# RoozbehSanaei/Structure-from-Motion-3D-Reconstruction

Hardware: NVIDIA B200
Metric: KLT feature-tracks/sec (+ RANSAC hyp*pts/sec under 'ransac') (higher is better)
Workload: dtype f64

## Files before the change

structure-from-motion-3d-reconstruction_b200/csrc/klt_lane.cu:

```cuda
#include "common.cuh"

namespace {

constexpr int LR = 5;
constexpr int LN = 2 * LR + 4;
constexpr int LNC = 2 * LR + 3;
constexpr int LIMG = LN * 16;
constexpr int LSTRIDE = 2 * LIMG + 16;
constexpr int LWARPS = 1;

__device__ __forceinline__ double byte_f64(uint32_t w, int k) {
  const uint32_t b = __byte_perm(w, 0, 0x4440 | k);
  double d;
  asm("cvt.rn.f64.u32 %0, %1;" : "=d"(d) : "r"(b));
  return d;
}

__device__ __forceinline__ void row_bytes(const uint4 q, double (&v)[LN]) {
  const uint32_t w[4] = {q.x, q.y, q.z, q.w};
#pragma unroll
  for (int i = 0; i < LN; i++) v[i] = byte_f64(w[i >> 2], i & 3);
}

template <int I0, int I1>
__device__ __forceinline__ void hlerp_row(const unsigned char* rowp, double fx, double (&h)[LNC]) {
  double px[LN];
  row_bytes(*reinterpret_cast<const uint4*>(rowp), px);
#pragma unroll
  for (int i = I0; i < I1; i++) h[i] = __fma_rn(fx, px[i + 1] - px[i], px[i]);
}

template <int ACC, bool MASKED>
__device__ __forceinline__ void walk_row(const unsigned char* tile, int v, double fx, double fy, unsigned cm, unsigned rm,
                                         double (&h1p)[LNC], double (&h0p)[LNC], const double (&sold)[LNC], const double (&smid)[LNC],
                                         double (&snew)[LNC], double (&acc)[ACC][5]) {
  double px[LN];
  row_bytes(*reinterpret_cast<const uint4*>(tile + v * 16), px);
  const unsigned cnew = MASKED ? (((rm >> (v - 1)) & 1u) ? cm : 0u) : 0u;
  const unsigned cpix = MASKED ? (((rm >> (v - 2)) & 1u) ? cm : 0u) : 0u;
#pragma unroll
  for (int i = 0; i < LNC; i++) {
    const double h = __fma_rn(fx, px[i + 1] - px[i], px[i]);
    double sn = __fma_rn(fy, h - h1p[i], h1p[i]);
    if (MASKED) sn = ((cnew >> i) & 1u) ? sn : 0.0;
    snew[i] = sn;
    h1p[i] = h;
  }
  row_bytes(*reinterpret_cast<const uint4*>(tile + LIMG + (v - 1) * 16), px);
#pragma unroll
  for (int i = 1; i <= LNC - 2; i++) {
    const double h = __fma_rn(fx, px[i + 1] - px[i], px[i]);
    double s0 = __fma_rn(fy, h - h0p[i], h0p[i]);
    if (MASKED) s0 = ((cpix >> i) & 1u) ? s0 : 0.0;
    h0p[i] = h;
    const double gx2 = smid[i + 1] - smid[i - 1];
    const double gy2 = snew[i] - sold[i];
    const double e = s0 - smid[i];
    double(&a)[5] = acc[i % ACC];
    a[0] = __fma_rn(gx2, gx2, a[0]);
    a[1] = __fma_rn(gx2, gy2, a[1]);
    a[2] = __fma_rn(gy2, gy2, a[2]);
    a[3] = __fma_rn(gx2, e, a[3]);
    a[4] = __fma_rn(gy2, e, a[4]);
  }
}

template <int ACC, bool MASKED>
__device__ __forceinline__ void window_sums(const unsigned char* tile, double fx, double fy, unsigned cm, unsigned rm, double& a00,
                                            double& a01, double& a11, double& b0, double& b1) {
  double h1p[LNC], h0p[LNC], s0[LNC], s1[LNC], s2[LNC], t[LNC];
  double acc[ACC][5];
#pragma unroll
  for (int j = 0; j < ACC; j++)
#pragma unroll
    for (int q = 0; q < 5; q++) acc[j][q] = 0.0;
  hlerp_row<0, LNC>(tile, fx, h1p);
  hlerp_row<0, LNC>(tile + 16, fx, t);
  const unsigned c0 = MASKED ? ((rm & 1u) ? cm : 0u) : 0u, c1 = MASKED ? ((rm & 2u) ? cm : 0u) : 0u;
#pragma unroll
  for (int i = 0; i < LNC; i++) {
    s0[i] = __fma_rn(fy, t[i] - h1p[i], h1p[i]);
    if (MASKED) s0[i] = ((c0 >> i) & 1u) ? s0[i] : 0.0;
    h1p[i] = t[i];
  }
  hlerp_row<0, LNC>(tile + 32, fx, t);
#pragma unroll
  for (int i = 0; i < LNC; i++) {
    s1[i] = __fma_rn(fy, t[i] - h1p[i], h1p[i]);
    if (MASKED) s1[i] = ((c1 >> i) & 1u) ? s1[i] : 0.0;
    h1p[i] = t[i];
  }
  hlerp_row<1, LNC - 1>(tile + LIMG + 16, fx, h0p);
#pragma unroll 1
  for (int v = 3; v < LN; v += 3) {
    walk_row<ACC, MASKED>(tile, v, fx, fy, cm, rm, h1p, h0p, s0, s1, s2, acc);
    walk_row<ACC, MASKED>(tile, v + 1, fx, fy, cm, rm, h1p, h0p, s1, s2, s0, acc);
    if (v + 2 < LN) walk_row<ACC, MASKED>(tile, v + 2, fx, fy, cm, rm, h1p, h0p, s2, s0, s1, acc);
  }
  a00 = acc[0][0]; a01 = acc[0][1]; a11 = acc[0][2]; b0 = acc[0][3]; b1 = acc[0][4];
#pragma unroll
  for (int j = 1; j < ACC; j++) {
    a00 += acc[j][0]; a01 += acc[j][1]; a11 += acc[j][2]; b0 += acc[j][3]; b1 += acc[j][4];
  }
}

struct StageRegs {
  uint4 lo, hi;
};

template <bool CLAMP>
__device__ __forceinline__ void stage_load(StageRegs& r, const uint8_t* __restrict__ imgA, const uint8_t* __restrict__ imgB, int pitch,
                                           int h, int x0, int y0, int lane) {
  const int img = lane >= LN ? 1 : 0, row = lane - img * LN;
  int y = y0 + row;
  if (CLAMP) y = y < 0 ? 0 : (y > h - 1 ? h - 1 : y);
  const uint8_t* rowp = (img ? imgA : imgB) + (size_t)y * pitch;
  const int xa = x0 & ~15, o = x0 & 15;
  int c0 = xa, c1 = xa + 16;
  if (CLAMP) {
    c0 = c0 < 0 ? 0 : (c0 > pitch - 16 ? pitch - 16 : c0);
    c1 = c1 < 0 ? 0 : (c1 > pitch - 16 ? pitch - 16 : c1);
  }
  r.lo = __ldg(reinterpret_cast<const uint4*>(rowp + c0));
  r.hi = make_uint4(0, 0, 0, 0);
  if (o > 2) r.hi = __ldg(reinterpret_cast<const uint4*>(rowp + c1));
}

__device__ __forceinline__ void stage_store(const StageRegs& r, unsigned char* tile_s, int x0, int lane) {
  const int img = lane >= LN ? 1 : 0, row = lane - img * LN;
  const int o = x0 & 15, q = o >> 2, sh = (o & 3) * 8;
  uint32_t W[8] = {r.lo.x, r.lo.y, r.lo.z, r.lo.w, r.hi.x, r.hi.y, r.hi.z, r.hi.w};
  if (q & 2) { W[0] = W[2]; W[1] = W[3]; W[2] = W[4]; W[3] = W[5]; W[4] = W[6]; W[5] = W[7]; }
  if (q & 1) { W[0] = W[1]; W[1] = W[2]; W[2] = W[3]; W[3] = W[4]; W[4] = W[5]; }
  uint4 out;
  out.x = __funnelshift_r(W[0], W[1], sh);
  out.y = __funnelshift_r(W[1], W[2], sh);
  out.z = __funnelshift_r(W[2], W[3], sh);
  out.w = __funnelshift_r(W[3], W[4], sh);
  *reinterpret_cast<uint4*>(tile_s + img * LIMG + row * 16) = out;
}

template <int ACC, int MINB, int LSTAGE, bool MASKED>
__global__ void __launch_bounds__(32 * LWARPS, MINB) klt_lane_kernel(KltLaunch k, const int* __restrict__ in_list,
                                                                     const int* __restrict__ in_count, int* __restrict__ defer_count,
                                                                     int* __restrict__ defer_list) {
  extern __shared__ __align__(16) unsigned char smem_raw[];
  const unsigned FULL = 0xffffffffu;
  const int warp = threadIdx.x >> 5, lane = threadIdx.x & 31;
  unsigned char* wtile = smem_raw + (size_t)warp * 32 * LSTRIDE;
  unsigned char* tile = wtile + lane * LSTRIDE;
  const long long total = (long long)k.npairs * k.cap;
  const long long nwork = MASKED ? (long long)*in_count : total;
  for (long long wbase = ((long long)blockIdx.x * LWARPS + warp) * 32; wbase < nwork; wbase += (long long)gridDim.x * LWARPS * 32) {
  const long long widx = wbase + lane;
  long long g = widx;
  if (MASKED) g = widx < nwork ? (long long)in_list[widx] : total;
  const int pair = g < total ? (int)(g / k.cap) : 0;
  const int slot = (int)(g - (long long)pair * k.cap);
  const bool valid = g < total && (!k.counts || slot < k.counts[pair]);

  double2 p0 = make_double2(0.0, 0.0);
  if (valid) p0 = k.p0[g];
  double px = p0.x, py = p0.y, x1 = 0.0, y1 = 0.0;
  int n_it = 0;
  bool alive = valid;
  const int ndir = k.pb ? 2 : 1;

  for (int dir = 0; dir < ndir; dir++) {
    for (int l = k.pv.levels - 1; l >= 0; --l) {
      const int w = k.pv.w[l], h = k.pv.h[l], pitch = k.pv.pitch[l];
      const uint8_t* lbase = k.pv.base[l];
      const size_t fstride = k.pv.fstride[l];
      const double scale = 1.0 / (double)(1 << l);
      const double plx = px * scale, ply = py * scale;
      double dlx = 0.0, dly = 0.0;
      bool done = !alive;
      int tFX = INT_MIN, tFY = INT_MIN;
      for (int it = 0; it < k.iters; ++it) {
        if (!__any_sync(FULL, !done)) break;
        const double x = plx + dlx, y = ply + dly;
        const double fxx = floor(x), fyy = floor(y);
        int FX = 0, FY = 0;
        unsigned cm = 0, rm = 0;
        bool act = !done;
        if (act) {
          const bool finite_ok = (fabs(fxx) < 1.0e9) && (fabs(fyy) < 1.0e9);
          FX = finite_ok ? (int)fxx : 0;
          FY = finite_ok ? (int)fyy : 0;
          bool ok;
          if (!MASKED) {
            ok = finite_ok && FX - LR - 1 >= 0 && FX + LR + 3 <= w - 1 && FY - LR - 1 >= 0 && FY + LR + 3 <= h - 1;
          } else {
            const double lim = 1.0 - 5.9604644775390625e-8;
            ok = finite_ok && w >= 16 && h >= 16 && (x - fxx) <= lim && (y - fyy) <= lim;
            if (ok) {
#pragma unroll
              for (int i = 0; i < LNC; i++) {
                const int cx = FX + i - LR - 1, cy = FY + i - LR - 1;
                cm |= (cx >= 0 && cx <= w - 2) ? (1u << i) : 0u;
                rm |= (cy >= 0 && cy <= h - 2) ? (1u << i) : 0u;
              }
            }
          }
          if (!ok) {
            alive = false;
            done = true;
            act = false;
          }
        }
        unsigned need = __ballot_sync(FULL, act && (FX != tFX || FY != tFY));
        if (need) {
          __syncwarp();
          while (need) {
            int ss[LSTAGE], sx0[LSTAGE];
            StageRegs sr[LSTAGE];
#pragma unroll
            for (int j = 0; j < LSTAGE; j++) {
              ss[j] = need ? __ffs(need) - 1 : -1;
              need &= need - 1;
              const int src = ss[j] < 0 ? 0 : ss[j];
              const int sFX = __shfl_sync(FULL, FX, src), sFY = __shfl_sync(FULL, FY, src), spair = __shfl_sync(FULL, pair, src);
              const int sA = k.fa0 + spair * k.fa_step, sB = k.fb0 + spair * k.fb_step;
              sx0[j] = sFX - LR - 1;
              if (ss[j] >= 0 && lane < 2 * LN)
                stage_load<MASKED>(sr[j], lbase + (size_t)(dir ? sB : sA) * fstride, lbase + (size_t)(dir ? sA : sB) * fstride, pitch, h,
                                   sx0[j], sFY - LR - 1, lane);
            }
#pragma unroll
            for (int j = 0; j < LSTAGE; j++)
              if (ss[j] >= 0 && lane < 2 * LN) stage_store(sr[j], wtile + ss[j] * LSTRIDE, sx0[j], lane);
          }
          __syncwarp();
        }
        if (act) {
          tFX = FX;
          tFY = FY;
          double a00, a01, a11, b0, b1;
          window_sums<ACC, MASKED>(tile, x - fxx, y - fyy, cm, rm, a00, a01, a11, b0, b1);
          double sx = 0.0, sy = 0.0;
          const double det = a00 * a11 - a01 * a01;
          if (!(fabs(det) < 16.0 * 1e-9)) {
            const double rd = 2.0 / det;
            sx = (a11 * b0 - a01 * b1) * rd;
            sy = (a00 * b1 - a01 * b0) * rd;
          }
          n_it++;
          dlx += sx;
          dly += sy;
          if (sfm_lk_step_small(sx, sy)) done = true;
        }
      }
      const double up = (double)(1 << l);
      px = (plx + dlx) * up;
      py = (ply + dly) * up;
    }
    if (dir == 0) {
      x1 = px;
      y1 = py;
    }
  }
  if (alive) {
    k.p1[g] = make_double2(x1, y1);
    if (k.pb) k.pb[g] = make_double2(px, py);
    if (k.nit) k.nit[g] = n_it;
    if (k.keep) {
      const double fbd = hypot(px - p0.x, py - p0.y);
      k.keep[g] = (fbd >= k.fb_thresh) ? 0 : 1;
    }
  }
  const unsigned dm = __ballot_sync(FULL, valid && !alive);
  if (dm) {
    int base = 0;
    if (lane == 0) base = atomicAdd(defer_count, __popc(dm));
    base = __shfl_sync(FULL, base, 0);
    if (valid && !alive) defer_list[base + __popc(dm & ((1u << lane) - 1u))] = (int)g;
  }
  __syncwarp();
  }
}


constexpr int QM = 50;
static_assert(QM * 8 <= 2 * LIMG, "the matrices alias the lane's tile");

template <typename T>
struct QuadFam {
  T m[10];
};

__device__ __forceinline__ int qmad(int a, int b, int c) { return a * b + c; }
__device__ __forceinline__ float qmad(float a, float b, float c) { return __fmaf_rn(a, b, c); }

template <bool SYM, typename T>
__device__ __forceinline__ void quad_same_row(QuadFam<T>& f, const T (&a)[12], const T (&b)[12], bool first, bool last) {
  const T p1 = a[0] * b[0], p12 = a[11] * b[11];
  T mid = a[1] * b[1];
#pragma unroll
  for (int c = 2; c < 11; c++) mid = qmad(a[c], b[c], mid);
  const T left = mid + p1, right = mid + p12;
  T rs01 = a[0] * b[1];
  if (!SYM) rs01 = qmad(b[0], a[1], rs01);
#pragma unroll
  for (int c = 1; c < 11; c++) {
    rs01 = qmad(a[c], b[c + 1], rs01);
    if (!SYM) rs01 = qmad(b[c], a[c + 1], rs01);
  }
  const T zero = (T)0;
  f.m[0] += last ? zero : left;
  f.m[4] += last ? zero : right;
  f.m[1] += last ? zero : rs01;
  f.m[7] += first ? zero : left;
  f.m[9] += first ? zero : right;
  f.m[8] += first ? zero : rs01;
}

template <bool SYM, typename T>
__device__ __forceinline__ void quad_cross_row(QuadFam<T>& f, const T (&ap)[12], const T (&bp)[12], const T (&ac)[12],
                                               const T (&bc)[12]) {
  T q1 = ap[0] * bc[0], q12 = ap[11] * bc[11], mid = ap[1] * bc[1];
  if (!SYM) {
    q1 = qmad(bp[0], ac[0], q1);
    q12 = qmad(bp[11], ac[11], q12);
    mid = qmad(bp[1], ac[1], mid);
  }
#pragma unroll
  for (int c = 2; c < 11; c++) {
    mid = qmad(ap[c], bc[c], mid);
    if (!SYM) mid = qmad(bp[c], ac[c], mid);
  }
  f.m[2] += mid + q1;
  f.m[6] += mid + q12;
  T m03 = f.m[3], m12 = f.m[5];
#pragma unroll
  for (int c = 0; c < 11; c++) {
    m03 = qmad(ap[c], bc[c + 1], m03);
    m12 = qmad(ap[c + 1], bc[c], m12);
    if (!SYM) {
      m03 = qmad(bp[c], ac[c + 1], m03);
      m12 = qmad(bp[c + 1], ac[c], m12);
    }
  }
  f.m[3] = m03;
  f.m[5] = m12;
}

template <bool SYM, typename T>
__device__ __forceinline__ void quad_store(const QuadFam<T>& f, double* m) {
#pragma unroll
  for (int e = 0; e < 10; e++) {
    const bool diag = e == 0 || e == 4 || e == 7 || e == 9;
    const double v = (double)f.m[e];
    m[e] = (SYM && !diag) ? v + v : v;
  }
}

__device__ __forceinline__ void row_vals(const uint4 q, int (&v)[LN]) {
  const uint32_t w[4] = {q.x, q.y, q.z, q.w};
#pragma unroll
  for (int i = 0; i < LN; i++) v[i] = (int)__byte_perm(w[i >> 2], 0, 0x4440 | (i & 3));
}
__device__ __forceinline__ void row_vals(const uint4 q, float (&v)[LN]) {
  const uint32_t w[4] = {q.x, q.y, q.z, q.w};
#pragma unroll
  for (int i = 0; i < LN; i++) v[i] = __uint_as_float(__byte_perm(w[i >> 2], 0x4B000000u, 0x7650 | (i & 3)));
}

template <typename T, int PASS>
__device__ __forceinline__ void quad_sweep(const unsigned char* tile, QuadFam<T>& f0, QuadFam<T>& f1, QuadFam<T>& f2) {
  constexpr bool NX = PASS != 2, NY = PASS != 1, NE = PASS != 0;
  T dxp[12], dyp[12], dep[12];
#pragma unroll
  for (int c = 0; c < 12; c++) dxp[c] = dyp[c] = dep[c] = (T)0;
#pragma unroll 1
  for (int rr = 1; rr <= 12; rr++) {
    T dxc[12], dyc[12], dec[12];
    {
      T t1c[LN];
      if (NX || NE) row_vals(*reinterpret_cast<const uint4*>(tile + rr * 16), t1c);
      if (NX) {
#pragma unroll
        for (int c = 1; c <= 12; c++) dxc[c - 1] = t1c[c + 1] - t1c[c - 1];
      }
      if (NE) {
        T t0[LN];
        row_vals(*reinterpret_cast<const uint4*>(tile + LIMG + rr * 16), t0);
#pragma unroll
        for (int c = 1; c <= 12; c++) dec[c - 1] = t0[c] - t1c[c];
      }
    }
    if (NY) {
      T t1m[LN], t1p[LN];
      row_vals(*reinterpret_cast<const uint4*>(tile + (rr - 1) * 16), t1m);
      row_vals(*reinterpret_cast<const uint4*>(tile + (rr + 1) * 16), t1p);
#pragma unroll
      for (int c = 1; c <= 12; c++) dyc[c - 1] = t1p[c] - t1m[c];
    }
    const bool first = rr == 1, last = rr == 12;
    if (PASS == 0) {
      quad_same_row<true>(f0, dxc, dxc, first, last);
      quad_same_row<true>(f1, dyc, dyc, first, last);
      quad_same_row<false>(f2, dxc, dyc, first, last);
      if (rr >= 2) {
        quad_cross_row<true>(f0, dxp, dxp, dxc, dxc);
        quad_cross_row<true>(f1, dyp, dyp, dyc, dyc);
        quad_cross_row<false>(f2, dxp, dyp, dxc, dyc);
      }
    } else if (PASS == 1) {
      quad_same_row<false>(f0, dxc, dec, first, last);
      if (rr >= 2) quad_cross_row<false>(f0, dxp, dep, dxc, dec);
    } else {
      quad_same_row<false>(f0, dyc, dec, first, last);
      if (rr >= 2) quad_cross_row<false>(f0, dyp, dep, dyc, dec);
    }
#pragma unroll
    for (int c = 0; c < 12; c++) {
      if (NX) dxp[c] = dxc[c];
      if (NY) dyp[c] = dyc[c];
      if (NE) dep[c] = dec[c];
    }
  }
}

template <typename T>
__device__ __forceinline__ void quad_build(const unsigned char* tile, double* m) {
  QuadFam<T> a, b, c, dummy;
#pragma unroll
  for (int e = 0; e < 10; e++) a.m[e] = b.m[e] = c.m[e] = (T)0;
  quad_sweep<T, 0>(tile, a, b, c);
  double r[30];
  quad_store<true>(a, r);
  quad_store<true>(b, r + 10);
  quad_store<false>(c, r + 20);
#pragma unroll
  for (int e = 0; e < 10; e++) a.m[e] = b.m[e] = (T)0;
  quad_sweep<T, 1>(tile, a, dummy, dummy);
  quad_sweep<T, 2>(tile, b, dummy, dummy);
#pragma unroll
  for (int e = 0; e < 30; e++) m[e] = r[e];
  quad_store<false>(a, m + 30);
  quad_store<false>(b, m + 40);
}

__device__ __forceinline__ void quad_eval(const double* m, double fx, double fy, double& a00, double& a01, double& a11, double& b0,
                                          double& b1) {
  const double gx = 1.0 - fx, gy = 1.0 - fy;
  const double w0 = gx * gy, w1 = fx * gy, w2 = gx * fy, w3 = fx * fy;
  const double ww[10] = {w0 * w0, w0 * w1, w0 * w2, w0 * w3, w1 * w1, w1 * w2, w1 * w3, w2 * w2, w2 * w3, w3 * w3};
  double s[5];
#pragma unroll
  for (int f = 0; f < 5; f++) {
    double mm[10];
#pragma unroll
    for (int q = 0; q < 5; q++) {
      const double2 t = *reinterpret_cast<const double2*>(m + f * 10 + 2 * q);
      mm[2 * q] = t.x;
      mm[2 * q + 1] = t.y;
    }
    double acc = mm[0] * ww[0];
#pragma unroll
    for (int q = 1; q < 10; q++) acc = __fma_rn(mm[q], ww[q], acc);
    s[f] = acc;
  }
  a00 = s[0];
  a11 = s[1];
  a01 = s[2];
  b0 = s[3];
  b1 = s[4];
}

#ifdef KLT_ROUND_STATS
__device__ unsigned long long klt_round_hist[2][33];
#endif

template <int MINB, int LSTAGE, typename T>
__global__ void __launch_bounds__(32, MINB) klt_quad_kernel(KltLaunch k, int* __restrict__ defer_count, int* __restrict__ defer_list) {
  extern __shared__ __align__(16) unsigned char smem_raw[];
  const unsigned FULL = 0xffffffffu;
  const int lane = threadIdx.x & 31;
  unsigned char* wtile = smem_raw;
  unsigned char* tile = wtile + lane * LSTRIDE;
  double* mq = reinterpret_cast<double*>(tile);
  const long long total = (long long)k.npairs * k.cap;
  const int ndir = k.pb ? 2 : 1;
  for (long long wbase = (long long)blockIdx.x * 32; wbase < total; wbase += (long long)gridDim.x * 32) {
    const long long g = wbase + lane;
    const int pair = g < total ? (int)(g / k.cap) : 0;
    const int slot = (int)(g - (long long)pair * k.cap);
    const bool valid = g < total && (!k.counts || slot < k.counts[pair]);
    double2 p0 = make_double2(0.0, 0.0);
    if (valid) p0 = k.p0[g];
    double px = p0.x, py = p0.y, x1 = 0.0, y1 = 0.0;
    int n_it = 0;
    bool alive = valid, finished = !valid;
    int dir = 0, l = k.pv.levels - 1, it = 0;
    bool leveldone = false;
    double plx = px * (1.0 / (double)(1 << l)), ply = py * (1.0 / (double)(1 << l)), dlx = 0.0, dly = 0.0;
    int tFX = INT_MIN, tFY = INT_MIN, tkey = -1;

    while (true) {
      if (!finished && (leveldone || it >= k.iters)) {
        const double up = (double)(1 << l);
        px = (plx + dlx) * up;
        py = (ply + dly) * up;
        if (l > 0) {
          l--;
        } else {
          if (dir == 0) {
            x1 = px;
            y1 = py;
          }
          dir++;
          l = k.pv.levels - 1;
          if (dir >= ndir) finished = true;
        }
        const double scale = 1.0 / (double)(1 << l);
        plx = px * scale;
        ply = py * scale;
        dlx = dly = 0.0;
        it = 0;
        leveldone = false;
      }
      if (!__any_sync(FULL, !finished)) break;
      const bool canwork = !finished && it < k.iters && !leveldone;
      const double x = plx + dlx, y = ply + dly;
      const double fxx = floor(x), fyy = floor(y);
      int FX = 0, FY = 0;
      bool act = canwork;
      if (act) {
        const int w = k.pv.w[l], h = k.pv.h[l];
        const bool finite_ok = (fabs(fxx) < 1.0e9) && (fabs(fyy) < 1.0e9);
        FX = finite_ok ? (int)fxx : 0;
        FY = finite_ok ? (int)fyy : 0;
        const bool ok = finite_ok && FX - LR - 1 >= 0 && FX + LR + 3 <= w - 1 && FY - LR - 1 >= 0 && FY + LR + 3 <= h - 1;
        if (!ok) {
          alive = false;
          finished = true;
          act = false;
        }
      }
      const int key = dir * SFM_MAXL + l;
      const bool hit = act && FX == tFX && FY == tFY && key == tkey;
#ifdef KLT_ROUND_STATS
      {
        const unsigned hm = __ballot_sync(FULL, hit);
        if (hm && lane == 0) atomicAdd(&klt_round_hist[1][__popc(hm)], 1ull);
      }
#endif
      if (__any_sync(FULL, hit)) {
        if (hit) {
          double a00, a01, a11, b0, b1;
          quad_eval(mq, x - fxx, y - fyy, a00, a01, a11, b0, b1);
          double sx = 0.0, sy = 0.0;
          const double det = a00 * a11 - a01 * a01;
          if (!(fabs(det) < 16.0 * 1e-9)) {
            const double rd = 2.0 / det;
            sx = (a11 * b0 - a01 * b1) * rd;
            sy = (a00 * b1 - a01 * b0) * rd;
          }
          n_it++;
          it++;
          dlx += sx;
          dly += sy;
          if (sfm_lk_step_small(sx, sy)) leveldone = true;
        }
        continue;
      }
      unsigned need = __ballot_sync(FULL, act);
      if (!need) continue;
#ifdef KLT_ROUND_STATS
      if (lane == 0) atomicAdd(&klt_round_hist[0][__popc(need)], 1ull);
#endif
      __syncwarp();
      while (need) {
        int ss[LSTAGE], sx0[LSTAGE];
        StageRegs sr[LSTAGE];
#pragma unroll
        for (int j = 0; j < LSTAGE; j++) {
          ss[j] = need ? __ffs(need) - 1 : -1;
          need &= need - 1;
          const int src = ss[j] < 0 ? 0 : ss[j];
          const int sFX = __shfl_sync(FULL, FX, src), sFY = __shfl_sync(FULL, FY, src), spair = __shfl_sync(FULL, pair, src);
          const int sl = __shfl_sync(FULL, l, src), sdir = __shfl_sync(FULL, dir, src);
          const int sA = k.fa0 + spair * k.fa_step, sB = k.fb0 + spair * k.fb_step;
          const uint8_t* lbase = k.pv.base[sl];
          const size_t fstride = k.pv.fstride[sl];
          sx0[j] = sFX - LR - 1;
          if (ss[j] >= 0 && lane < 2 * LN)
            stage_load<false>(sr[j], lbase + (size_t)(sdir ? sB : sA) * fstride, lbase + (size_t)(sdir ? sA : sB) * fstride,
                              k.pv.pitch[sl], k.pv.h[sl], sx0[j], sFY - LR - 1, lane);
        }
#pragma unroll
        for (int j = 0; j < LSTAGE; j++)
          if (ss[j] >= 0 && lane < 2 * LN) stage_store(sr[j], wtile + ss[j] * LSTRIDE, sx0[j], lane);
      }
      __syncwarp();
      if (act) {
        quad_build<T>(tile, mq);
        tFX = FX;
        tFY = FY;
        tkey = key;
      }
      __syncwarp();
    }
    if (alive) {
      k.p1[g] = make_double2(x1, y1);
      if (k.pb) k.pb[g] = make_double2(px, py);
      if (k.nit) k.nit[g] = n_it;
      if (k.keep) {
        const double fbd = hypot(px - p0.x, py - p0.y);
        k.keep[g] = (fbd >= k.fb_thresh) ? 0 : 1;
      }
    }
    const unsigned dm = __ballot_sync(FULL, valid && !alive);
    if (dm) {
      int base = 0;
      if (lane == 0) base = atomicAdd(defer_count, __popc(dm));
      base = __shfl_sync(FULL, base, 0);
      if (valid && !alive) defer_list[base + __popc(dm & ((1u << lane) - 1u))] = (int)g;
    }
    __syncwarp();
  }
}

}

template <int ACC, int MINB, int LSTAGE, bool MASKED>
static int lane_launch(sfmgpu_ctx* ctx, const KltLaunch& k, const int* in_list, const int* in_count, int* defer_count, int* defer_list) {
  const size_t smem = (size_t)LWARPS * 32 * LSTRIDE;
  static const int cfg_id = sfm_next_cfg_id();
  SFM_SMEM_OPTIN(ctx, cfg_id, (klt_lane_kernel<ACC, MINB, LSTAGE, MASKED>), smem);
  const long long total = (long long)k.npairs * k.cap;
  if (total == 0) return 0;
  unsigned grid = sfm_cdiv(total, 32 * LWARPS);
  if (MASKED) {
    const unsigned cap = (unsigned)ctx->n_sm * 8;
    grid = grid < cap ? grid : cap;
  }
  SFM_LAUNCH(ctx, (klt_lane_kernel<ACC, MINB, LSTAGE, MASKED>), grid, 32 * LWARPS, smem, k, in_list, in_count, defer_count, defer_list);
  return 0;
}

template <int MINB, int LSTAGE, typename T>
static int quad_launch(sfmgpu_ctx* ctx, const KltLaunch& k, int* defer_count, int* defer_list) {
  const size_t smem = (size_t)32 * LSTRIDE;
  static const int cfg_id = sfm_next_cfg_id();
  SFM_SMEM_OPTIN(ctx, cfg_id, (klt_quad_kernel<MINB, LSTAGE, T>), smem);
  const long long total = (long long)k.npairs * k.cap;
  if (total == 0) return 0;
  SFM_LAUNCH(ctx, (klt_quad_kernel<MINB, LSTAGE, T>), sfm_cdiv(total, 32), 32, smem, k, defer_count, defer_list);
  return 0;
}

int sfm_klt_lane_launch(sfmgpu_ctx* ctx, const KltLaunch& k, int* defer_count, int* defer_list, int variant) {
  switch (variant) {
    case 1: return lane_launch<1, 12, 4, false>(ctx, k, nullptr, nullptr, defer_count, defer_list);
    case 2: return lane_launch<2, 8, 4, false>(ctx, k, nullptr, nullptr, defer_count, defer_list);
    case 3: return lane_launch<1, 8, 4, false>(ctx, k, nullptr, nullptr, defer_count, defer_list);
    case 4: return quad_launch<8, 4, int>(ctx, k, defer_count, defer_list);
    case 5: return quad_launch<8, 4, float>(ctx, k, defer_count, defer_list);
    case 6: return quad_launch<12, 4, float>(ctx, k, defer_count, defer_list);
    default: return quad_launch<12, 2, float>(ctx, k, defer_count, defer_list);
  }
}

int sfm_klt_lane_masked_launch(sfmgpu_ctx* ctx, const KltLaunch& k, const int* in_list, const int* in_count, int* defer_count,
                               int* defer_list) {
  return lane_launch<1, 8, 4, true>(ctx, k, in_list, in_count, defer_count, defer_list);
}

#ifdef KLT_ROUND_STATS
extern "C" int sfmgpu_debug_klt_round_hist(unsigned long long* out66) {
  return (int)cudaMemcpyFromSymbol(out66, klt_round_hist, sizeof(unsigned long long) * 66);
}
#endif
```

Before: 81.19 million.

## Build KLT quad moment tables with fp16 tensor-core MMA instead of per-lane sweeps

Adds a TcBuild path that stages per-feature gradient differences as fp16 in shared memory and computes the quadratic moment sums with ldmatrix plus mma.m16n8k16, one tile at a time across the warp. The results are scattered back to the per-lane tile as doubles. This path becomes the default variant, replacing the scalar float quad_build. It adds shared memory, serialises tiles across the warp, and lowers intermediate precision to fp16 inputs with fp32 accumulation.

```diff
diff --git a/structure-from-motion-3d-reconstruction_b200/csrc/klt_lane.cu b/structure-from-motion-3d-reconstruction_b200/csrc/klt_lane.cu
--- a/structure-from-motion-3d-reconstruction_b200/csrc/klt_lane.cu
+++ b/structure-from-motion-3d-reconstruction_b200/csrc/klt_lane.cu
@@ -441,6 +441,113 @@
   quad_store<false>(b, m + 40);
 }
 
+struct TcBuild {};
+constexpr int TC_STAGE = 161 * 16;
+constexpr int TC_CBUF = (16 * 8 + 4) * 4;
+__device__ __forceinline__ int tc_block(int fd) {
+  return fd == 0 ? 0 : (fd == 1 ? 25 : (fd == 2 ? 53 : (fd == 3 ? 84 : (fd == 4 ? 112 : 137))));
+}
+
+__device__ __forceinline__ uint32_t h2_sub(uint32_t a, uint32_t b) {
+  uint32_t d;
+  asm("sub.rn.f16x2 %0, %1, %2;" : "=r"(d) : "r"(a), "r"(b));
+  return d;
+}
+
+__device__ __forceinline__ void tc_magic_pairs(const uint4 q, int o, uint32_t (&h)[6]) {
+  const uint32_t w[4] = {q.x, q.y, q.z, q.w};
+#pragma unroll
+  for (int i = 0; i < 3; i++) {
+    const uint32_t s = __funnelshift_r(w[i], w[i + 1], 8 * o);
+    h[2 * i] = __byte_perm(s, 0x64646464u, 0x4140);
+    h[2 * i + 1] = __byte_perm(s, 0x64646464u, 0x4342);
+  }
+}
+
+__device__ __forceinline__ void tc_line(const unsigned char* tile, int f, int R, uint32_t (&d)[6]) {
+  const int prow = f == 0 ? R * 16 : (f == 1 ? (R + 1) * 16 : LIMG + R * 16);
+  const int qrow = f == 1 ? (R - 1) * 16 : R * 16;
+  uint32_t p[6], q[6];
+  tc_magic_pairs(*reinterpret_cast<const uint4*>(tile + prow), f == 0 ? 2 : 1, p);
+  tc_magic_pairs(*reinterpret_cast<const uint4*>(tile + qrow), f == 0 ? 0 : 1, q);
+#pragma unroll
+  for (int j = 0; j < 6; j++) d[j] = h2_sub(p[j], q[j]);
+}
+
+__device__ __forceinline__ void tc_line_store(unsigned char* stg, int f, int R, const uint32_t (&d)[6]) {
+  uint4* l0 = reinterpret_cast<uint4*>(stg + (tc_block(2 * f) + 2 * (R - 1)) * 16);
+  uint4* l1 = reinterpret_cast<uint4*>(stg + (tc_block(2 * f + 1) + 2 * (R - 1)) * 16);
+  l0[0] = make_uint4(d[0], d[1], d[2], d[3]);
+  *reinterpret_cast<uint2*>(l0 + 1) = make_uint2(d[4], d[5] & 0xffffu);
+  l1[0] = make_uint4(__byte_perm(d[0], d[1], 0x5432), __byte_perm(d[1], d[2], 0x5432), __byte_perm(d[2], d[3], 0x5432),
+                     __byte_perm(d[3], d[4], 0x5432));
+  *reinterpret_cast<uint2*>(l1 + 1) = make_uint2(__byte_perm(d[4], d[5], 0x5432), d[5] >> 16);
+}
+
+__device__ __forceinline__ void tc_stage(const unsigned char* tile, unsigned char* stg, int lane) {
+  const int f = lane < 24 ? (lane >> 2 & 1) : 2, R = lane < 24 ? 4 * (lane >> 3) + (lane & 3) + 1 : lane - 23;
+  uint32_t d[6], e[6];
+  tc_line(tile, f, R, d);
+  tc_line(tile, 2, 9 + (lane & 3), e);
+  tc_line_store(stg, f, R, d);
+  if (lane < 4) tc_line_store(stg, 2, 9 + lane, e);
+}
+
+__device__ __forceinline__ uint32_t tc_entry(int e) {
+  const int F = e / 10, i = e - 10 * F;
+  const int k = i < 4 ? 0 : (i < 7 ? 1 : (i < 9 ? 2 : 3));
+  const int l = k + i - (k == 0 ? 0 : (k == 1 ? 4 : (k == 2 ? 7 : 9)));
+  int a, b;
+  switch (F) {
+    case 0: a = k * 8 + l; b = a; break;
+    case 1: a = (4 + k) * 8 + 4 + l; b = a; break;
+    case 2: a = k * 8 + 4 + l; b = l * 8 + 4 + k; break;
+    case 3: a = (8 + l) * 8 + k; b = (8 + k) * 8 + l; break;
+    default: a = (8 + l) * 8 + 4 + k; b = (8 + k) * 8 + 4 + l;
+  }
+  if (k == l) b = 128;
+  return (uint32_t)a | ((uint32_t)b << 8);
+}
+
+__device__ __forceinline__ void tc_build(unsigned char* wtile, unsigned char* stg, float* cbuf, unsigned need, int lane,
+                                         uint32_t a_base, uint32_t ent) {
+  int s = __ffs(need) - 1;
+  need &= need - 1;
+  tc_stage(wtile + s * LSTRIDE, stg, lane);
+  while (true) {
+    __syncwarp();
+    float c[4][4] = {};
+#pragma unroll
+    for (int r = 1; r <= 11; r++) {
+      uint32_t a0, a1, a2, a3;
+      asm volatile("ldmatrix.sync.aligned.m8n8.x4.shared.b16 {%0, %1, %2, %3}, [%4];"
+                   : "=r"(a0), "=r"(a1), "=r"(a2), "=r"(a3)
+                   : "r"(a_base + 32 * r)
+                   : "memory");
+      float(&d)[4] = c[r & 3];
+      asm("mma.sync.aligned.m16n8k16.row.col.f32.f16.f16.f32 {%0, %1, %2, %3}, {%4, %5, %6, %7}, {%8, %9}, {%0, %1, %2, %3};"
+          : "+f"(d[0]), "+f"(d[1]), "+f"(d[2]), "+f"(d[3])
+          : "r"(a0), "r"(a1), "r"(a2), "r"(a3), "r"(a0), "r"(a2));
+    }
+    float v[4];
+#pragma unroll
+    for (int q = 0; q < 4; q++) v[q] = (c[0][q] + c[1][q]) + (c[2][q] + c[3][q]);
+    const int g = lane >> 2, t = lane & 3;
+    *reinterpret_cast<float2*>(cbuf + g * 8 + 2 * t) = make_float2(v[0], v[1]);
+    *reinterpret_cast<float2*>(cbuf + (g + 8) * 8 + 2 * t) = make_float2(v[2], v[3]);
+    __syncwarp();
+    const int sn = need ? __ffs(need) - 1 : -1;
+    need &= need - 1;
+    if (lane < 25) {
+      const float v0 = cbuf[ent & 0xff] + cbuf[(ent >> 8) & 0xff], v1 = cbuf[(ent >> 16) & 0xff] + cbuf[ent >> 24];
+      reinterpret_cast<double2*>(wtile + s * LSTRIDE)[lane] = make_double2((double)v0, (double)v1);
+    }
+    if (sn < 0) break;
+    tc_stage(wtile + sn * LSTRIDE, stg, lane);
+    s = sn;
+  }
+}
+
 __device__ __forceinline__ void quad_eval(const double* m, double fx, double fy, double& a00, double& a01, double& a11, double& b0,
                                           double& b1) {
   const double gx = 1.0 - fx, gy = 1.0 - fy;
@@ -474,12 +581,24 @@
 
 template <int MINB, int LSTAGE, typename T>
 __global__ void __launch_bounds__(32, MINB) klt_quad_kernel(KltLaunch k, int* __restrict__ defer_count, int* __restrict__ defer_list) {
+  constexpr bool TC = std::is_same<T, TcBuild>::value;
   extern __shared__ __align__(16) unsigned char smem_raw[];
   const unsigned FULL = 0xffffffffu;
   const int lane = threadIdx.x & 31;
   unsigned char* wtile = smem_raw;
   unsigned char* tile = wtile + lane * LSTRIDE;
   double* mq = reinterpret_cast<double*>(tile);
+  unsigned char* stg = wtile + 32 * LSTRIDE;
+  float* cbuf = reinterpret_cast<float*>(stg + TC_STAGE);
+  uint32_t a_base = 0, ent = 0;
+  if (TC) {
+    int m = (lane >> 3 & 1) * 8 + (lane & 7);
+    if (m >= 12) m -= 4;
+    a_base = (uint32_t)__cvta_generic_to_shared(stg) + (tc_block(2 * (m >> 2) + (m & 1)) + 2 * ((m >> 1 & 1) - 1) + (lane >> 4)) * 16;
+    if (lane < 25) ent = tc_entry(2 * lane) | tc_entry(2 * lane + 1) << 16;
+    for (int i = lane; i < (TC_STAGE + TC_CBUF) / 16; i += 32) reinterpret_cast<uint4*>(stg)[i] = make_uint4(0u, 0u, 0u, 0u);
+    __syncwarp();
+  }
   const long long total = (long long)k.npairs * k.cap;
   const int ndir = k.pb ? 2 : 1;
   for (long long wbase = (long long)blockIdx.x * 32; wbase < total; wbase += (long long)gridDim.x * 32) {
@@ -571,6 +690,7 @@
       if (lane == 0) atomicAdd(&klt_round_hist[0][__popc(need)], 1ull);
 #endif
       __syncwarp();
+      const unsigned build = need;
       while (need) {
         int ss[LSTAGE], sx0[LSTAGE];
         StageRegs sr[LSTAGE];
@@ -594,8 +714,9 @@
           if (ss[j] >= 0 && lane < 2 * LN) stage_store(sr[j], wtile + ss[j] * LSTRIDE, sx0[j], lane);
       }
       __syncwarp();
+      if constexpr (TC) tc_build(wtile, stg, cbuf, build, lane, a_base, ent);
       if (act) {
-        quad_build<T>(tile, mq);
+        if constexpr (!TC) quad_build<T>(tile, mq);
         tFX = FX;
         tFY = FY;
         tkey = key;
@@ -642,7 +763,7 @@
 
 template <int MINB, int LSTAGE, typename T>
 static int quad_launch(sfmgpu_ctx* ctx, const KltLaunch& k, int* defer_count, int* defer_list) {
-  const size_t smem = (size_t)32 * LSTRIDE;
+  const size_t smem = (size_t)32 * LSTRIDE + (std::is_same<T, TcBuild>::value ? TC_STAGE + TC_CBUF : 0);
   static const int cfg_id = sfm_next_cfg_id();
   SFM_SMEM_OPTIN(ctx, cfg_id, (klt_quad_kernel<MINB, LSTAGE, T>), smem);
   const long long total = (long long)k.npairs * k.cap;
@@ -659,7 +780,8 @@
     case 4: return quad_launch<8, 4, int>(ctx, k, defer_count, defer_list);
     case 5: return quad_launch<8, 4, float>(ctx, k, defer_count, defer_list);
     case 6: return quad_launch<12, 4, float>(ctx, k, defer_count, defer_list);
-    default: return quad_launch<12, 2, float>(ctx, k, defer_count, defer_list);
+    case 7: return quad_launch<12, 2, float>(ctx, k, defer_count, defer_list);
+    default: return quad_launch<12, 2, TcBuild>(ctx, k, defer_count, defer_list);
   }
 }
 
```

Result: slower. 78.22 million, median of 6 (-3.7%).

## Build KLT quadratic moments via u8 IMMA Gram matrix on tensor cores

Applied to the files above, without the earlier changes.

Adds a GramBuild path to the quad kernel. Each active lane's patch is packed into u8 tap vectors, and one Gram matrix per tile is computed with mma.sync m16n8k32 u8 instructions. The quadratic-form moments are then recovered as signed combinations of Gram entries, instead of the per-lane scalar float or int sweeps. The default variant switches to this path with MINB 14. It serialises the tile builds across the warp, adds shared scratch, and masks the staged tile's last word.

```diff
diff --git a/structure-from-motion-3d-reconstruction_b200/csrc/klt_lane.cu b/structure-from-motion-3d-reconstruction_b200/csrc/klt_lane.cu
--- a/structure-from-motion-3d-reconstruction_b200/csrc/klt_lane.cu
+++ b/structure-from-motion-3d-reconstruction_b200/csrc/klt_lane.cu
@@ -1,3 +1,5 @@
+#include <type_traits>
+
 #include "common.cuh"
 
 namespace {
@@ -136,7 +138,7 @@
   out.x = __funnelshift_r(W[0], W[1], sh);
   out.y = __funnelshift_r(W[1], W[2], sh);
   out.z = __funnelshift_r(W[2], W[3], sh);
-  out.w = __funnelshift_r(W[3], W[4], sh);
+  out.w = __funnelshift_r(W[3], W[4], sh) & 0xFFFFu;
   *reinterpret_cast<uint4*>(tile_s + img * LIMG + row * 16) = out;
 }
 
@@ -441,6 +443,127 @@
   quad_store<false>(b, m + 40);
 }
 
+struct GramBuild {};
+constexpr int GRAM_SCRATCH = 3 * 256;
+constexpr int ZROW = 2 * LIMG;
+
+__device__ __forceinline__ void gram_tap(int j, int& dr, int& dc, int& img) {
+  if (j < 8) { dr = j >> 2; dc = (j & 3) - 1; img = 0; }
+  else if (j < 12) { dr = j < 10 ? -1 : 2; dc = j & 1; img = 0; }
+  else { dr = (j - 12) >> 1; dc = j & 1; img = 1; }
+}
+
+__device__ __forceinline__ int gram_diff_tap(int side, int k, bool plus) {
+  const int a = k >> 1, b = k & 1;
+  if (side == 0) return a * 4 + b + (plus ? 2 : 0);
+  if (side == 1) return plus ? (a ? 10 + b : 5 + b) : (a ? 1 + b : 8 + b);
+  return plus ? 12 + 2 * a + b : a * 4 + b + 1;
+}
+
+__device__ __forceinline__ int gram_at(int i, int j) {
+  if (i >= 8 && j < 8) { const int s = i; i = j; j = s; }
+  return i < 8 ? (j < 8 ? (i * 8 + j) * 4 : 256 + (i * 8 + j - 8) * 4) : 512 + ((i - 8) * 8 + j - 8) * 4;
+}
+
+struct GramLane {
+  int rb[2], r2[2];
+  uint32_t sel[2], selm[2];
+  int ga[2][8];
+};
+
+__device__ __forceinline__ void gram_lane_init(GramLane& L, int lane, int zero_off) {
+  const int g = lane >> 2, t = lane & 3;
+#pragma unroll
+  for (int x = 0; x < 2; x++) {
+    int dr, dc, img;
+    gram_tap(g + 8 * x, dr, dc, img);
+    L.rb[x] = img * LIMG + (dr + t + 1) * 16;
+    L.r2[x] = t == 3 ? ZROW : L.rb[x] + 128;
+    L.sel[x] = 0x3210u + 0x1111u * (uint32_t)(dc + 1);
+    L.selm[x] = (L.sel[x] & 0x0FFFu) | 0x7000u;
+  }
+#pragma unroll
+  for (int h = 0; h < 2; h++) {
+    const int e = lane + 32 * h, f = e / 10, q = e % 10;
+    const int k = q < 4 ? 0 : q < 7 ? 1 : q < 9 ? 2 : 3;
+    const int l = k + q - (q < 4 ? 0 : q < 7 ? 4 : q < 9 ? 7 : 9);
+    const int sa = (f == 1 || f == 4) ? 1 : 0, sb = f == 0 ? 0 : f <= 2 ? 1 : 2;
+#pragma unroll
+    for (int d = 0; d < 2; d++) {
+      const int ka = d ? l : k, kb = d ? k : l;
+      const int ap = gram_diff_tap(sa, ka, true), am = gram_diff_tap(sa, ka, false);
+      const int bp = gram_diff_tap(sb, kb, true), bm = gram_diff_tap(sb, kb, false);
+      const bool z = e >= QM || (d == 1 && k == l);
+      L.ga[h][4 * d + 0] = z ? zero_off : gram_at(ap, bp);
+      L.ga[h][4 * d + 1] = z ? zero_off : gram_at(ap, bm);
+      L.ga[h][4 * d + 2] = z ? zero_off : gram_at(am, bp);
+      L.ga[h][4 * d + 3] = z ? zero_off : gram_at(am, bm);
+    }
+  }
+}
+
+template <int U>
+__device__ __forceinline__ uint32_t gram_word(const unsigned char* ftile, const GramLane& L, int x) {
+  constexpr int CLS = U / 3, J = U % 3;
+  if (U >= 9) return 0u;
+  const unsigned char* rowp = ftile + (J == 2 ? L.r2[x] : L.rb[x] + 64 * J);
+  const uint32_t sel = CLS == 2 ? L.selm[x] : L.sel[x];
+  if (CLS == 1) {
+    const uint4 q = *reinterpret_cast<const uint4*>(rowp);
+    return __byte_perm(q.y, q.z, sel);
+  }
+  const uint2 q = *reinterpret_cast<const uint2*>(rowp + 4 * CLS);
+  return __byte_perm(q.x, q.y, sel);
+}
+
+__device__ __forceinline__ void imma_16832(int (&d)[4], uint32_t a0, uint32_t a1, uint32_t a2, uint32_t a3, uint32_t b0, uint32_t b1) {
+  asm("mma.sync.aligned.m16n8k32.row.col.s32.u8.u8.s32 {%0,%1,%2,%3}, {%4,%5,%6,%7}, {%8,%9}, {%0,%1,%2,%3};"
+      : "+r"(d[0]), "+r"(d[1]), "+r"(d[2]), "+r"(d[3])
+      : "r"(a0), "r"(a1), "r"(a2), "r"(a3), "r"(b0), "r"(b1));
+}
+
+__device__ __forceinline__ void gram_build(unsigned char* ftile, unsigned char* scratch, const GramLane& L, int lane) {
+  uint32_t w[2][10];
+#pragma unroll
+  for (int x = 0; x < 2; x++) {
+    w[x][0] = gram_word<0>(ftile, L, x);
+    w[x][1] = gram_word<1>(ftile, L, x);
+    w[x][2] = gram_word<2>(ftile, L, x);
+    w[x][3] = gram_word<3>(ftile, L, x);
+    w[x][4] = gram_word<4>(ftile, L, x);
+    w[x][5] = gram_word<5>(ftile, L, x);
+    w[x][6] = gram_word<6>(ftile, L, x);
+    w[x][7] = gram_word<7>(ftile, L, x);
+    w[x][8] = gram_word<8>(ftile, L, x);
+    w[x][9] = gram_word<9>(ftile, L, x);
+  }
+  int d0[4] = {0, 0, 0, 0}, d1[4] = {0, 0, 0, 0};
+#pragma unroll
+  for (int s = 0; s < 5; s++) {
+    const uint32_t a0 = w[0][2 * s], a1 = w[1][2 * s], a2 = w[0][2 * s + 1], a3 = w[1][2 * s + 1];
+    imma_16832(d0, a0, a1, a2, a3, a0, a2);
+    imma_16832(d1, a0, a1, a2, a3, a1, a3);
+  }
+  const int o = (lane >> 2) * 8 + 2 * (lane & 3);
+  int* G = reinterpret_cast<int*>(scratch);
+  *reinterpret_cast<int2*>(G + o) = make_int2(d0[0], d0[1]);
+  *reinterpret_cast<int2*>(G + 64 + o) = make_int2(d1[0], d1[1]);
+  *reinterpret_cast<int2*>(G + 128 + o) = make_int2(d1[2], d1[3]);
+  __syncwarp();
+#pragma unroll
+  for (int h = 0; h < 2; h++) {
+    const int e = lane + 32 * h;
+    if (e < QM) {
+      const int* a = L.ga[h];
+#define GR(i) (*reinterpret_cast<const int*>(scratch + a[i]))
+      const int v = (GR(0) - GR(1) - GR(2) + GR(3)) + (GR(4) - GR(5) - GR(6) + GR(7));
+#undef GR
+      reinterpret_cast<double*>(ftile)[e] = (double)v;
+    }
+  }
+  __syncwarp();
+}
+
 __device__ __forceinline__ void quad_eval(const double* m, double fx, double fy, double& a00, double& a01, double& a11, double& b0,
                                           double& b1) {
   const double gx = 1.0 - fx, gy = 1.0 - fy;
@@ -482,6 +605,13 @@
   double* mq = reinterpret_cast<double*>(tile);
   const long long total = (long long)k.npairs * k.cap;
   const int ndir = k.pb ? 2 : 1;
+  constexpr bool GRAM = std::is_same<T, GramBuild>::value;
+  unsigned char* scratch = smem_raw + 32 * LSTRIDE;
+  GramLane gl;
+  if (GRAM) {
+    gram_lane_init(gl, lane, ZROW - 32 * LSTRIDE);
+    *reinterpret_cast<uint4*>(tile + ZROW) = make_uint4(0u, 0u, 0u, 0u);
+  }
   for (long long wbase = (long long)blockIdx.x * 32; wbase < total; wbase += (long long)gridDim.x * 32) {
     const long long g = wbase + lane;
     const int pair = g < total ? (int)(g / k.cap) : 0;
@@ -570,6 +700,7 @@
 #ifdef KLT_ROUND_STATS
       if (lane == 0) atomicAdd(&klt_round_hist[0][__popc(need)], 1ull);
 #endif
+      const unsigned build = need;
       __syncwarp();
       while (need) {
         int ss[LSTAGE], sx0[LSTAGE];
@@ -594,8 +725,12 @@
           if (ss[j] >= 0 && lane < 2 * LN) stage_store(sr[j], wtile + ss[j] * LSTRIDE, sx0[j], lane);
       }
       __syncwarp();
+      if constexpr (GRAM) {
+        for (unsigned todo = build; todo; todo &= todo - 1) gram_build(wtile + (__ffs(todo) - 1) * LSTRIDE, scratch, gl, lane);
+      } else if (act) {
+        quad_build<T>(tile, mq);
+      }
       if (act) {
-        quad_build<T>(tile, mq);
         tFX = FX;
         tFY = FY;
         tkey = key;
@@ -642,7 +777,7 @@
 
 template <int MINB, int LSTAGE, typename T>
 static int quad_launch(sfmgpu_ctx* ctx, const KltLaunch& k, int* defer_count, int* defer_list) {
-  const size_t smem = (size_t)32 * LSTRIDE;
+  const size_t smem = (size_t)32 * LSTRIDE + (std::is_same<T, GramBuild>::value ? GRAM_SCRATCH : 0);
   static const int cfg_id = sfm_next_cfg_id();
   SFM_SMEM_OPTIN(ctx, cfg_id, (klt_quad_kernel<MINB, LSTAGE, T>), smem);
   const long long total = (long long)k.npairs * k.cap;
@@ -659,7 +794,9 @@
     case 4: return quad_launch<8, 4, int>(ctx, k, defer_count, defer_list);
     case 5: return quad_launch<8, 4, float>(ctx, k, defer_count, defer_list);
     case 6: return quad_launch<12, 4, float>(ctx, k, defer_count, defer_list);
-    default: return quad_launch<12, 2, float>(ctx, k, defer_count, defer_list);
+    case 7: return quad_launch<12, 2, float>(ctx, k, defer_count, defer_list);
+    case 8: return quad_launch<12, 2, GramBuild>(ctx, k, defer_count, defer_list);
+    default: return quad_launch<14, 2, GramBuild>(ctx, k, defer_count, defer_list);
   }
 }
 
```

After: 81.18 million before, 83.95 million after (median of 6 runs). +3.4%, better.
